# christopherkarani/Wax

Hardware: NVIDIA H100
Metric: queries/sec cosine top-10 @ 10Mx384 fp32 (higher is better)
Workload: dtype f32

## Files before the change

### wax_b200/csrc/waxvs_batch.cuh

```cuda
#pragma once
#include <cuda.h>
#include <cuda_bf16.h>

#include "waxvs_common.cuh"
#include "waxvs_scan.cuh"

namespace waxvs {

constexpr int kBatchM = 128;
constexpr int kBatchN = 128;
constexpr int kBatchKBlock = 32;
constexpr int kBatchKBlockBf16 = 64;
constexpr int kBatchRescore = 256;
constexpr int kBatchRescoreMax = 1024;
constexpr uint32_t kBatchABytes = kBatchM * 128u;
constexpr uint32_t kBatchBBytes = kBatchN * 128u;
constexpr uint32_t kBatchStageBytes = kBatchABytes + kBatchBBytes;
constexpr int kBatchStageSlots = 8;
constexpr uint32_t kBatchScoreStride = kBatchN + 8;
constexpr uint32_t kBatchScoreBytes = kBatchM * kBatchScoreStride * 4u;
constexpr int kBatchMaxStages = 6;
constexpr uint32_t kBatchSmemOptin = 227u * 1024u;
__host__ __device__ constexpr uint32_t batch_smem_bytes(int stages, int heap, uint32_t ares_kb = 0) {
    return ares_kb * kBatchABytes + stages * (ares_kb ? kBatchBBytes : kBatchStageBytes) + kBatchScoreBytes +
// ... 590 lines not shown
}

template <int METRIC>
__device__ __forceinline__ float exact_row_distance(const float *q, const float *v, uint32_t dims, float a2,
                                                    float sqrt_a2, int lane) {
    float a0 = 0.f, a1 = 0.f, a2_ = 0.f, a3 = 0.f, b0 = 0.f, b1 = 0.f, b2 = 0.f, b3 = 0.f;
    auto acc = [&](float qx, float vx, float &a, float &b) {
        if (METRIC == kL2) { const float dd = __fsub_rn(qx, vx); a = __fmaf_rn(dd, dd, a); }
        else { a = __fmaf_rn(qx, vx, a); if (METRIC == kCosine) b = __fmaf_rn(vx, vx, b); }
    };
    if ((dims % 4u) == 0u) {
        const float4 *v4 = reinterpret_cast<const float4 *>(v);
        const float4 *q4 = reinterpret_cast<const float4 *>(q);
        for (uint32_t c = lane; c < dims / 4u; c += 32u) {
            const float4 x = __ldg(v4 + c), y = __ldg(q4 + c);
            acc(y.x, x.x, a0, b0); acc(y.y, x.y, a1, b1); acc(y.z, x.z, a2_, b2); acc(y.w, x.w, a3, b3);
        }
    } else {
        for (uint32_t base = 4u * lane; base < dims; base += 128u) {
            acc(__ldg(q + base), __ldg(v + base), a0, b0);
            if (base + 1 < dims) acc(__ldg(q + base + 1), __ldg(v + base + 1), a1, b1);
            if (base + 2 < dims) acc(__ldg(q + base + 2), __ldg(v + base + 2), a2_, b2);
            if (base + 3 < dims) acc(__ldg(q + base + 3), __ldg(v + base + 3), a3, b3);
        }
    }
    const float s0 = warp_butterfly_sum(__fadd_rn(__fadd_rn(a0, a1), __fadd_rn(a2_, a3)));
    if (METRIC == kCosine) {
        const float s1 = warp_butterfly_sum(__fadd_rn(__fadd_rn(b0, b1), __fadd_rn(b2, b3)));
        return finish_cos(s0, a2, sqrt_a2, s1);
    }
    return METRIC == kDot ? finish_dot(s0) : finish_l2(s0);
}

template <int METRIC>
__device__ __forceinline__ void exact_row_distance_x4(const float *q, const float *const (&v)[4], uint32_t dims, float a2,
                                                      float sqrt_a2, int lane, float (&d)[4]) {
    if ((dims % 4u) != 0u) {
#pragma unroll
        for (int r = 0; r < 4; ++r) d[r] = exact_row_distance<METRIC>(q, v[r], dims, a2, sqrt_a2, lane);
        return;
    }
    float a[4][4], b[4][4];
#pragma unroll
    for (int r = 0; r < 4; ++r)
#pragma unroll
        for (int j = 0; j < 4; ++j) { a[r][j] = 0.f; b[r][j] = 0.f; }
    auto acc = [&](float qx, float vx, float &aa, float &bb) {
        if (METRIC == kL2) { const float dd = __fsub_rn(qx, vx); aa = __fmaf_rn(dd, dd, aa); }
        else { aa = __fmaf_rn(qx, vx, aa); if (METRIC == kCosine) bb = __fmaf_rn(vx, vx, bb); }
    };
    const float4 *q4 = reinterpret_cast<const float4 *>(q);
    for (uint32_t c = lane; c < dims / 4u; c += 32u) {
        float4 x[4];
#pragma unroll
        for (int r = 0; r < 4; ++r) x[r] = __ldg(reinterpret_cast<const float4 *>(v[r]) + c);
        const float4 y = __ldg(q4 + c);
#pragma unroll
        for (int r = 0; r < 4; ++r) {
            acc(y.x, x[r].x, a[r][0], b[r][0]); acc(y.y, x[r].y, a[r][1], b[r][1]);
            acc(y.z, x[r].z, a[r][2], b[r][2]); acc(y.w, x[r].w, a[r][3], b[r][3]);
        }
    }
#pragma unroll
    for (int r = 0; r < 4; ++r) {
        const float s0 = warp_butterfly_sum(__fadd_rn(__fadd_rn(a[r][0], a[r][1]), __fadd_rn(a[r][2], a[r][3])));
        if (METRIC == kCosine) {
            const float s1 = warp_butterfly_sum(__fadd_rn(__fadd_rn(b[r][0], b[r][1]), __fadd_rn(b[r][2], b[r][3])));
            d[r] = finish_cos(s0, a2, sqrt_a2, s1);
        } else {
            d[r] = METRIC == kDot ? finish_dot(s0) : finish_l2(s0);
        }
    }
}

__device__ __forceinline__ void block_bitonic_sort(uint64_t *sk, uint32_t pow2) {
    for (uint32_t size = 2; size <= pow2; size <<= 1) {
        for (uint32_t stride = size >> 1; stride > 0; stride >>= 1) {
            for (uint32_t i = threadIdx.x; i < pow2 / 2; i += blockDim.x) {
                const uint32_t lo = (i / stride) * (2 * stride) + (i % stride), hi = lo + stride;
                const bool asc = ((lo & size) == 0);
                const uint64_t a = sk[lo], b = sk[hi];
                if ((a > b) == asc) { sk[lo] = b; sk[hi] = a; }
            }
            __syncthreads();
        }
    }
}

template <int METRIC>
__global__ void __launch_bounds__(256) gather_score_kernel(const float *corpus, const float *queries, uint32_t dims,
                                                           const uint32_t *rows_all, const uint2 *span, uint32_t key_stride,
                                                           uint64_t *keys_all) {
    const int lane = threadIdx.x & 31;
// ... 105 lines not shown
                                         float eps_rel, bool excluded_any, uint32_t &ok, float &tau_star,
                                         float &tau_star16) {
    const float n = static_cast<float>(dims);
    const float delta = (n + 4.0f) * 0x1p-23f;
    const float one_m = __fsub_rd(1.0f, delta), one_p = __fadd_ru(1.0f, delta);
    const float qn = __fmul_ru(sqrt_a2, one_p);
    const float em = l2_nomination_bound(eps_rel, qn, max_norm, n);
    const float a_lo = __fsub_rd(__fmul_rd(a2, one_m), 1e-30f);
    float lhs = __fsub_rd(a_lo, __fmul_ru(2.0f, __fadd_ru(tau, em)));
    lhs = __fsub_rd(__fmul_rd(__fmul_rd(lhs, one_m), __fsub_rd(1.0f, 0x1p-20f)), 1e-30f);
    if (excluded_any && (!(lhs > dk) || !finite_f32(lhs) || !finite_f32(em) || !finite_f32(a2))) ok = 0;
    const float a_lo_f = __fsub_rd(__fdiv_rd(a2, one_p), 1e-30f);
    const float d_hi = __fadd_ru(__fdiv_ru(dk, one_m), 1e-30f);
    auto threshold = [&](float eps) {
        const float e = l2_nomination_bound(eps, qn, max_norm, n);
        const float t = __fsub_rd(__fmul_rd(0.5f, __fsub_rd(a_lo_f, d_hi)), e);
        return (finite_f32(t) && finite_f32(e) && finite_f32(a2)) ? t - fabsf(t) * 0x1p-20f - 1e-30f : -INFINITY;
    };
    tau_star = threshold(kTf32Eps);
    tau_star16 = threshold(kBf16Eps);
}

template <int METRIC>
__global__ void __launch_bounds__(512, 2) batch_finish_kernel(const FinishParams p) {
    extern __shared__ uint64_t fsm[];
    uint64_t *sk = fsm;
    uint64_t *ek = fsm + p.pow2_all;
    __shared__ float s_a2, s_sqrt_a2;
    __shared__ uint32_t s_valid, s_excl;
    const uint32_t q = blockIdx.x, g = q / kBatchM, t = q % kBatchM;
    const int warp = threadIdx.x >> 5, lane = threadIdx.x & 31;
    const float *qv = p.queries + static_cast<size_t>(q) * p.dims;

    if (threadIdx.x == 0) { s_valid = 0; s_excl = 0; }
    __syncthreads();
    const uint32_t total = p.slices * p.kprime;
    uint32_t cnt = 0;
    for (uint32_t i = threadIdx.x; i < p.pow2_all; i += blockDim.x) {
        uint64_t key = WAXVS_KEY_NONE;
        if (i < total) {
            const uint32_t s = i / p.kprime, e = i % p.kprime;
            key = p.heaps[(static_cast<size_t>(s * p.groups + g) * p.kprime + e) * kBatchM + t];
            if (key != WAXVS_KEY_NONE) {
                ++cnt;
                if (e == 0) atomicMax(&s_excl, orderable_u32(nominee_score(key)));
            }
        }
        sk[i] = key;
    }
    if (cnt) atomicAdd(&s_valid, cnt);
    if (warp == 0) {
        float s0 = 0.f, s1 = 0.f, s2 = 0.f, s3 = 0.f;
        for (uint32_t base = 4u * lane; base < p.dims; base += 128u) {
            const float x = __ldg(qv + base); s0 = __fmaf_rn(x, x, s0);
            if (base + 1 < p.dims) { const float y = __ldg(qv + base + 1); s1 = __fmaf_rn(y, y, s1); }
            if (base + 2 < p.dims) { const float z = __ldg(qv + base + 2); s2 = __fmaf_rn(z, z, s2); }
            if (base + 3 < p.dims) { const float w = __ldg(qv + base + 3); s3 = __fmaf_rn(w, w, s3); }
        }
        const float a2 = warp_butterfly_sum(__fadd_rn(__fadd_rn(s0, s1), __fadd_rn(s2, s3)));
        if (lane == 0) { s_a2 = a2; s_sqrt_a2 = __fsqrt_rn(a2); }
    }
    __syncthreads();
    block_bitonic_sort(sk, p.pow2_all);

    const uint32_t n_valid = s_valid;
    const uint32_t kpp = min(p.rescore, n_valid);
    float tau = s_excl ? from_orderable_u32(s_excl) : -INFINITY;
// ... 55 lines not shown
            ok = 0;
        }
        if (METRIC != kL2 && (!(s_a2 >= 0x1p-126f) || !finite_f32(s_a2))) {
            ok = 0;
            tau_star = tau_star16 = -INFINITY;
        }
        p.ok[q] = ok;
        if (p.tau_star) { p.tau_star[q] = tau_star; p.tau_star[p.tau_stride + q] = tau_star16; }
    }
    ScanParams sp{};
    sp.out = p.out + static_cast<size_t>(q) * p.k;
    sp.frame_ids = p.frame_ids; sp.id_base = p.id_base; sp.row_offset = p.row_offset;
    for (uint32_t i = threadIdx.x; i < p.k; i += blockDim.x)
        write_candidate(sp, static_cast<int>(i), i < p.rescore ? ek[i] : WAXVS_KEY_NONE);
}

struct RescoreParams {
    const float *corpus, *query;
    uint32_t dims, k, n_nominees;
    const uint64_t *nominees;
    uint32_t *aux;
    const uint32_t *max_norm_bits;
    float rho_max;
    uint64_t *block_keys;
    uint32_t *ticket;
    uint32_t *work_counter;
    wax_vs_candidate *out;
    uint32_t *ok;
    const uint64_t *frame_ids;
    uint64_t id_base, row_offset;
    uint32_t tail_smem_bytes;
};

template <int METRIC>
__global__ void __launch_bounds__(512, 1) shadow_rescore_kernel(const RescoreParams p) {
    static_assert(METRIC == kCosine || METRIC == kDot, "the shadow route covers cosine and dot");
    extern __shared__ __align__(16) unsigned char rsm[];
    __shared__ float s_a2, s_sqrt_a2;
    const int warp = threadIdx.x >> 5, lane = threadIdx.x & 31, warps = blockDim.x >> 5;
    const int k = static_cast<int>(p.k);
    if (warp == 0) {
        float s0 = 0.f, s1 = 0.f, s2 = 0.f, s3 = 0.f;
        for (uint32_t base = 4u * lane; base < p.dims; base += 128u) {
            const float4 x = __ldg(reinterpret_cast<const float4 *>(p.query + base));
            s0 = __fmaf_rn(x.x, x.x, s0); s1 = __fmaf_rn(x.y, x.y, s1);
            s2 = __fmaf_rn(x.z, x.z, s2); s3 = __fmaf_rn(x.w, x.w, s3);
        }
        const float a2 = warp_butterfly_sum(__fadd_rn(__fadd_rn(s0, s1), __fadd_rn(s2, s3)));
        if (lane == 0) { s_a2 = a2; s_sqrt_a2 = __fsqrt_rn(a2); }
    }
    __shared__ ScanParams sp;
    for (uint32_t i = threadIdx.x; i < sizeof(ScanParams) / 4u; i += blockDim.x) reinterpret_cast<uint32_t *>(&sp)[i] = 0u;
    __syncthreads();
    if (threadIdx.x == 0) {
        sp.k = p.k; sp.block_keys = p.block_keys; sp.ticket = p.ticket; sp.out = p.out;
        sp.frame_ids = p.frame_ids; sp.id_base = p.id_base; sp.row_offset = p.row_offset;
        sp.tail_smem_bytes = p.tail_smem_bytes; sp.work_counter = p.work_counter;
    }
    __syncthreads();

    WarpTopK<1> tk;
    tk.init();
    const uint32_t stride = gridDim.x * warps * 4u;
    for (uint32_t i0 = (blockIdx.x * warps + warp) * 4u; i0 < p.n_nominees; i0 += stride) {
        uint64_t nk[4];
        const float *vp[4];
        float d[4];
#pragma unroll
        for (uint32_t r = 0; r < 4; ++r) {
            nk[r] = i0 + r < p.n_nominees ? p.nominees[i0 + r] : WAXVS_KEY_NONE;
            vp[r] = p.corpus + static_cast<size_t>(nk[r] == WAXVS_KEY_NONE ? 0u : static_cast<uint32_t>(nk[r])) * p.dims;
        }
        exact_row_distance_x4<METRIC>(p.query, vp, p.dims, s_a2, s_sqrt_a2, lane, d);
#pragma unroll
        for (uint32_t r = 0; r < 4; ++r) {
            if (nk[r] == WAXVS_KEY_NONE || !finite_f32(d[r])) continue;
            const uint64_t x = make_key(d[r], static_cast<uint32_t>(nk[r]));
            if (x < tk.thresh) tk.insert(x, lane, k);
        }
    }

    if (!finish_topk_select<1>(sp, tk, rsm)) return;
    __syncthreads();
    if (threadIdx.x != 0) return;
    const wax_vs_candidate kth = p.out[p.k - 1];
    const uint32_t cut = p.aux[0];
    const bool excluded_any = cut != WAXVS_UKEY_NONE;
    const float tau = excluded_any ? -from_orderable_u32(cut) : -INFINITY;
    const float rho_q = __uint_as_float(p.aux[1]);
    uint32_t ok = 1;
    if (kth.valid) {
        const float dk = kth.distance, qn = s_sqrt_a2;
        const float m = METRIC == kCosine ? 1.0f : __uint_as_float(*p.max_norm_bits);
        const float scale = qn * m;
        const float sk_exact = METRIC == kCosine ? (1.0f - dk) * qn : 1.0f - dk;
        const float coding = qn * p.rho_max + rho_q * ((METRIC == kCosine ? 1.0001f : m) + p.rho_max);
        const float acc_slack = static_cast<float>(p.dims) * 0x1p-23f * scale;
        const float ulp_slack = 0x1p-21f * fmaxf(1.0f, fabsf(dk)) * (METRIC == kCosine ? qn : 1.0f);
        const float eps = coding * 1.01f + acc_slack + ulp_slack + 1e-30f;
        if (excluded_any && (!(sk_exact > tau + eps) || !finite_f32(eps))) ok = 0;
    } else if (excluded_any) {
        ok = 0;
    }
    if (!(s_a2 >= 0x1p-126f) || !finite_f32(s_a2)) ok = 0;
    *p.ok = ok;
    p.aux[0] = WAXVS_UKEY_NONE;
    p.aux[2] = cut;
}

template <int METRIC>
__global__ void __launch_bounds__(256) filter_rescore_kernel(const float *corpus, const float *queries, uint32_t dims,
                                                             const uint32_t *cand_count, const uint32_t *cand_rows,
// ... 71 lines not shown
```

### wax_b200/csrc/waxvs_common.cuh

```cuda
#pragma once
#include <cuda_runtime.h>
#include <stdint.h>

#define WAXVS_KEY_NONE 0xFFFFFFFFFFFFFFFFull
#define WAXVS_UKEY_NONE 0xFFFFFFFFu
#define WAXVS_FULL_MASK 0xFFFFFFFFu

namespace waxvs {

enum Metric : int { kCosine = 0, kDot = 1, kL2 = 2 };

__device__ __forceinline__ uint32_t orderable_u32(float f) {
    uint32_t u = __float_as_uint(f);
    return u ^ ((u & 0x80000000u) ? 0xFFFFFFFFu : 0x80000000u);
}
__device__ __forceinline__ float from_orderable_u32(uint32_t k) {
    uint32_t u = k ^ ((k & 0x80000000u) ? 0x80000000u : 0xFFFFFFFFu);
    return __uint_as_float(u);
}
__host__ __device__ __forceinline__ bool finite_f32(float f) {
#ifdef __CUDA_ARCH__
    return (__float_as_uint(f) & 0x7F800000u) != 0x7F800000u;
#else
    union { float f; uint32_t u; } x; x.f = f;
// ... 225 lines not shown
            "selp.u32 %0, 1, 0, p;\n\t}"
            : "=r"(done)
            : "r"(addr), "r"(parity)
            : "memory");
    } while (!done);
}
__device__ __forceinline__ void bulk_copy_g2s(void *smem_dst, const void *gmem_src, uint32_t bytes,
                                              uint64_t *bar) {
    asm volatile(
        "cp.async.bulk.shared::cluster.global.mbarrier::complete_tx::bytes [%0], [%1], %2, [%3];" ::"r"(
            smem_u32(smem_dst)),
        "l"(gmem_src), "r"(bytes), "r"(smem_u32(bar))
        : "memory");
}
__device__ __forceinline__ void bulk_copy_g2s_hint(void *smem_dst, const void *gmem_src, uint32_t bytes,
                                                   uint64_t *bar, uint64_t policy) {
    asm volatile(
        "cp.async.bulk.shared::cluster.global.mbarrier::complete_tx::bytes.L2::cache_hint [%0], [%1], %2, "
        "[%3], %4;" ::"r"(smem_u32(smem_dst)),
        "l"(gmem_src), "r"(bytes), "r"(smem_u32(bar)), "l"(policy)
        : "memory");
}
__device__ __forceinline__ uint64_t l2_policy_evict_first() {
    uint64_t pol;
    asm volatile("createpolicy.fractional.L2::evict_first.b64 %0, 1.0;" : "=l"(pol));
    return pol;
}
__device__ __forceinline__ uint64_t ld_cg_u64(const uint64_t *p) {
    uint64_t v;
    asm volatile("ld.global.cg.u64 %0, [%1];" : "=l"(v) : "l"(p) : "memory");
    return v;
}

}
```

### wax_b200/csrc/waxvs_engine.cu

```cuda
#include <cuda_runtime.h>

#include <algorithm>
#include <atomic>
#include <cstdarg>
#include <cstdio>
#include <cstring>
#include <limits>
#include <map>
#include <mutex>
#include <new>
#include <shared_mutex>
#include <string>
#include <unordered_map>
#include <chrono>
#include <random>
#include <thread>
#include <unistd.h>
#include <cmath>
#include <vector>

#include "../../include/wax_vs_cuda.h"
#include "waxvs_common.cuh"
#include "waxvs_scan.cuh"
#include "waxvs_select.cuh"
// ... 113 lines not shown
enum RouteForm : int { kRouteBf16, kRouteInt8, kRouteU4, kRouteForms };

struct Tuning {
    int variant = 0;
    int rows_per_step = 0;
    int stages = 0;
    int warps = 0;
    int grid = 0;
    int l2_hint = 0;
    int ldg_ctas_per_sm = 4;
    int chunk_steps = -1;
    int fused_k_max = 128;
    int batch_tensor = 1;
    int batch_min = 4;
    int time_overlap = 0;
    int batch_pair = 0;
    uint32_t tma_max_dims = 4096;
    int batch_large_k = 1;
    int batch_heap = 0;
    int batch_noinsert = 0;
    int batch_bf16 = 1;
    int batch_ares = 1;
    int batch_rescore = 0;
    int batch_retry = 1;
    int filter_bf16 = 1;
    int filter_cap = 8192;
    int inline_query = 1;
    int host_delivery = 1;
    int tail_select = 1;
    int shard_fused = 1;
    int batch_l2 = 0;
    int single_shadow = 0;
    uint64_t filter_bitset_bytes = 2ull << 30;
    int shadow_scan = 1;
    struct Route { uint64_t min_bytes; int rows_per_step = 0, warps = 0, stages = 0; };
    Route route[kRouteForms] = {
        {512ull << 20},
        {512ull << 20},
        {2048ull << 20},
    };
};

struct SearchCtx {
    cudaStream_t stream = nullptr;
    bool own_stream = false;
    DevBuf<float> d_queries;
    DevBuf<wax_vs_candidate> d_out;
    PinnedBuf<float> h_queries;
    PinnedBuf<wax_vs_candidate> h_out;
    DevBuf<uint64_t> d_block_keys;
    DevBuf<uint32_t> d_ticket;
    DevBuf<uint32_t> d_dist_keys;
    DevBuf<SelectState> d_select;
    DevBuf<uint64_t> d_sel_keys;
    cudaEvent_t ev0 = nullptr, ev1 = nullptr;
    DevBuf<uint64_t> d_heaps;
    DevBuf<uint32_t> d_ok;
    PinnedBuf<uint32_t> h_ok;
    DevBuf<uint32_t> d_tau;
    DevBuf<__nv_bfloat16> d_queries_bf16;
    DevBuf<float> d_retry_q;
    DevBuf<wax_vs_candidate> d_retry_out;
    DevBuf<uint32_t> d_retry_ok;
    DevBuf<float> d_tau_star;
    PinnedBuf<float> h_tau_star;
    DevBuf<float> d_filter_tau;
// ... 335 lines not shown
    } else if (C == 12) {
        R = e->tune.rows_per_step == 1 || e->tune.rows_per_step == 2 ? e->tune.rows_per_step : 2;
    } else if (C >= 6) {
        R = e->tune.rows_per_step == 2 || e->tune.rows_per_step == 4 ? e->tune.rows_per_step : 2;
    } else {
        R = e->tune.rows_per_step == 4 || e->tune.rows_per_step == 8 ? e->tune.rows_per_step : (C <= 2 ? 8 : 4);
        if (C == 1) warps_default = 16;
        else if (C == 2) warps_default = 12;
        else if (mode == 1 && static_cast<uint64_t>(e->n_rows) * d * 4 < (8ull << 30)) warps_default = 16;
    }
    const int stages = e->tune.stages > 0 ? e->tune.stages : 2;
    const size_t stage_bytes = static_cast<size_t>(R) * d * sizeof(float);
    const size_t query_bytes = C == 0 ? (static_cast<size_t>(d) * 4 + 512 + 32) : 0;
    auto smem_for = [&](int w) { return tma_ring_smem(w, stages, stage_bytes) + query_bytes; };
    int warps = std::max(1, std::min(16, e->tune.warps ? e->tune.warps : warps_default));
    if (!e->tune.warps) while (warps > 2 && smem_for(warps) > budget) --warps;
    if (smem_for(warps) > budget) return false;
    cfg->C = C; cfg->R = R; cfg->warps = warps; cfg->stages = stages; cfg->smem = smem_for(warps);
    return true;
}

template <typename K>
static cudaError_t grant_smem(wax_vs_engine *e, K kernel, size_t bytes) {
    static std::mutex mu;
    static std::map<std::pair<int, const void *>, int> granted;
    std::lock_guard<std::mutex> g(mu);
    int &have = granted[{e->device, reinterpret_cast<const void *>(kernel)}];
    if (have >= static_cast<int>(bytes)) return cudaSuccess;
    cudaError_t err = cudaFuncSetAttribute(kernel, cudaFuncAttributeMaxDynamicSharedMemorySize, static_cast<int>(bytes));
    if (err == cudaSuccess) have = static_cast<int>(bytes);
    return err;
}

template <int C, int R, int M, int E, bool EMIT, bool SHADOW = false, bool INT8 = false, bool U4 = false>
static cudaError_t launch_tma_inst(wax_vs_engine *e, const ScanParams &p, int grid, const TmaConfig &cfg, cudaStream_t s) {
    cudaError_t err = grant_smem(e, scan_tma_kernel<C, R, M, E, EMIT, SHADOW, INT8, U4>, cfg.smem);
    if (err != cudaSuccess) return err;
    scan_tma_kernel<C, R, M, E, EMIT, SHADOW, INT8, U4><<<grid, cfg.warps * 32, cfg.smem, s>>>(p);
    return cudaGetLastError();
}
template <int C, int R>
static cudaError_t launch_tma_cr(wax_vs_engine *e, const ScanParams &p, int grid, const TmaConfig &cfg, int metric, int mode,
                                 cudaStream_t s) {
    switch (metric * 3 + mode) {
        case 0: return launch_tma_inst<C, R, kCosine, 1, false>(e, p, grid, cfg, s);
        case 1: return launch_tma_inst<C, R, kCosine, 4, false>(e, p, grid, cfg, s);
        case 2: return launch_tma_inst<C, R, kCosine, 1, true>(e, p, grid, cfg, s);
        case 3: return launch_tma_inst<C, R, kDot, 1, false>(e, p, grid, cfg, s);
        case 4: return launch_tma_inst<C, R, kDot, 4, false>(e, p, grid, cfg, s);
        case 5: return launch_tma_inst<C, R, kDot, 1, true>(e, p, grid, cfg, s);
        case 6: return launch_tma_inst<C, R, kL2, 1, false>(e, p, grid, cfg, s);
        case 7: return launch_tma_inst<C, R, kL2, 4, false>(e, p, grid, cfg, s);
        default: return launch_tma_inst<C, R, kL2, 1, true>(e, p, grid, cfg, s);
    }
}
static cudaError_t launch_tma(wax_vs_engine *e, const ScanParams &p, int grid, const TmaConfig &cfg, int metric, int mode,
                              cudaStream_t s) {
#define WAXVS_CASE(Cv, Rv) if (cfg.C == Cv && cfg.R == Rv) return launch_tma_cr<Cv, Rv>(e, p, grid, cfg, metric, mode, s)
    WAXVS_CASE(1, 4); WAXVS_CASE(1, 8); WAXVS_CASE(2, 4); WAXVS_CASE(2, 8);
    WAXVS_CASE(3, 4); WAXVS_CASE(3, 8); WAXVS_CASE(4, 4); WAXVS_CASE(4, 8);
    WAXVS_CASE(6, 2); WAXVS_CASE(6, 4); WAXVS_CASE(8, 2); WAXVS_CASE(8, 4);
    WAXVS_CASE(12, 1); WAXVS_CASE(12, 2);
    WAXVS_CASE(0, 1); WAXVS_CASE(0, 2); WAXVS_CASE(0, 4); WAXVS_CASE(0, 8);
#undef WAXVS_CASE
    return cudaErrorInvalidValue;
}
template <RouteForm F, int C, int R>
static cudaError_t launch_route_cr(wax_vs_engine *e, const ScanParams &p, int grid, const TmaConfig &cfg, int metric,
                                   cudaStream_t s) {
    if constexpr (F == kRouteU4) {
        return launch_tma_inst<C, R, kDot, 4, false, true, false, true>(e, p, grid, cfg, s);
    } else {
        return metric == kCosine ? launch_tma_inst<C, R, kCosine, 4, false, true, F == kRouteInt8>(e, p, grid, cfg, s)
                                 : launch_tma_inst<C, R, kDot, 4, false, true, F == kRouteInt8>(e, p, grid, cfg, s);
    }
}
#define WAXVS_CASE(Cv, Rv) \
    if (cfg.C == Cv && cfg.R == Rv) return p ? launch_route_cr<F, Cv, Rv>(e, *p, grid, cfg, metric, s) : cudaSuccess
static cudaError_t launch_shadow_scan(wax_vs_engine *e, const ScanParams *p, int grid, const TmaConfig &cfg, int metric,
                                      cudaStream_t s) {
    constexpr RouteForm F = kRouteBf16;
    WAXVS_CASE(1, 8); WAXVS_CASE(1, 16); WAXVS_CASE(2, 8); WAXVS_CASE(2, 16);
    WAXVS_CASE(3, 4); WAXVS_CASE(3, 8); WAXVS_CASE(3, 16); WAXVS_CASE(4, 4); WAXVS_CASE(4, 8);
    WAXVS_CASE(6, 2); WAXVS_CASE(6, 4); WAXVS_CASE(8, 2); WAXVS_CASE(8, 4); WAXVS_CASE(12, 2); WAXVS_CASE(12, 4);
    return cudaErrorInvalidValue;
}
static cudaError_t launch_int8_scan(wax_vs_engine *e, const ScanParams *p, int grid, const TmaConfig &cfg, int metric,
                                   cudaStream_t s) {
    constexpr RouteForm F = kRouteInt8;
    WAXVS_CASE(1, 8); WAXVS_CASE(1, 16); WAXVS_CASE(2, 8); WAXVS_CASE(2, 16);
    WAXVS_CASE(3, 4); WAXVS_CASE(3, 8); WAXVS_CASE(3, 16); WAXVS_CASE(4, 4); WAXVS_CASE(4, 8);
// ... 143 lines not shown

static bool batch_bf16_wanted(const wax_vs_engine *e);
static int32_t ensure_shadow(wax_vs_engine *e, cudaStream_t stream);
static int32_t ensure_coded_shadow(wax_vs_engine *e, RouteForm f, cudaStream_t stream, bool keep_coarse);
static int32_t ensure_route_shadow(wax_vs_engine *e, RouteForm f, cudaStream_t stream, bool keep_coarse = false) {
    return f == kRouteBf16 ? ensure_shadow(e, stream) : ensure_coded_shadow(e, f, stream, keep_coarse);
}

constexpr uint32_t kShadowNominees = 128;
constexpr uint32_t kShadowRescore = 256;
constexpr uint32_t kShadowSkipQueries = 16;
static bool shadow_route_applies(const wax_vs_engine *e) {
    return e->tune.shadow_scan && (e->similarity == WAX_VS_COSINE || e->similarity == WAX_VS_DOT) && !e->debug_trace &&
           e->tune.batch_bf16 != 0 && e->dims % kBatchKBlockBf16 == 0 &&
           e->n_rows * e->dims * sizeof(float) >= e->tune.route[kRouteBf16].min_bytes;
}
static int32_t select_route_form(wax_vs_engine *e, cudaStream_t stream, bool demoted, bool *use, RouteForm *form,
                                 TmaConfig *cfg) {
    *use = false;
    for (const RouteForm f : {kRouteU4, kRouteInt8, kRouteBf16}) {
        if ((f == kRouteU4 && demoted) || e->n_rows * e->dims * sizeof(float) < e->tune.route[f].min_bytes ||
            !pick_route_config(e, f, cfg))
            continue;
        if (const int32_t rc = ensure_route_shadow(e, f, stream)) return rc;
        if (e->shadows[f].valid && e->shadows[f].eps_rel <= kRouteSpec[f].max_eps_rel) {
            *use = true;
            *form = f;
            return WAX_VS_OK;
        }
    }
    return WAX_VS_OK;
}

static int32_t enqueue_shadow_nominations(wax_vs_engine *e, SearchCtx *c, const ScanParams &p, const TmaConfig &cfg,
                                          cudaStream_t stream, uint64_t *launches, uint32_t *shape, RouteForm f) {
    const RouteFormSpec &fs = kRouteSpec[f];
    const wax_vs_engine::Shadow &sh = e->shadows[f];
    int32_t rc;
    if (fs.grid_rescore && !c->d_u4_aux) {
        if ((rc = c->d_u4_aux.ensure(3, "4-bit route state"))) return rc;
        CUDA_TRY(cudaMemsetAsync(c->d_u4_aux, 0xFF, 3 * sizeof(uint32_t), stream));
    }
    const size_t cta_keys = static_cast<size_t>(std::max(e->tune.grid, e->sm_count)) * kU4CtaNominees;
    if ((rc = c->d_heaps.ensure(std::max(static_cast<size_t>(kShadowNominees) * kNomineeStride, fs.grid_rescore ? cta_keys : 0), "nominee keys")) ||
        (rc = c->d_ok.ensure(1, "proof flags")) || (!p.query && (rc = c->d_queries.ensure(e->dims, "query buffer"))))
        return rc;

    ScanParams sp = p;
    sp.corpus = reinterpret_cast<const float *>(sh.codes.p);
    sp.row_scale = fs.scaled ? sh.scale.p : nullptr;
    sp.u4_aux = fs.grid_rescore ? c->d_u4_aux.p : nullptr;
    sp.k = kShadowNominees;
    sp.out = nullptr; sp.host_out = nullptr; sp.host_flag = nullptr;
    sp.nominees = c->d_heaps;
    sp.query_store = p.query ? nullptr : c->d_queries.p;
    sp.tail_select = e->tune.tail_select ? 1u : 0u;
    sp.tail_smem_bytes = static_cast<uint32_t>(static_cast<size_t>(cfg.warps) * cfg.stages * cfg.R * e->dims * fs.tail_bytes);
    const int grid = tma_grid(e, c, cfg, sp);
    CUDA_TRY(fs.launch(e, &sp, grid, cfg, e->similarity, stream));

    if (fs.grid_rescore) {
        RescoreParams rp{};
        rp.corpus = e->d_corpus; rp.query = p.query ? p.query : c->d_queries.p;
        rp.dims = e->dims; rp.k = p.k; rp.n_nominees = static_cast<uint32_t>(grid) * kU4CtaNominees;
        rp.nominees = c->d_heaps; rp.aux = c->d_u4_aux; rp.max_norm_bits = e->d_max_norm; rp.rho_max = sh.rho_max;
        rp.block_keys = c->d_block_keys; rp.ticket = c->d_ticket; rp.work_counter = sp.work_counter; rp.out = p.out; rp.ok = c->d_ok;
        rp.frame_ids = p.frame_ids; rp.id_base = p.id_base; rp.row_offset = p.row_offset;
        rp.tail_smem_bytes = static_cast<uint32_t>(grid) * p.k * sizeof(uint64_t);
        if (rp.tail_smem_bytes > 48u * 1024u) rp.tail_smem_bytes = 0;
        const auto kernel = e->similarity == WAX_VS_COSINE ? shadow_rescore_kernel<kCosine> : shadow_rescore_kernel<kDot>;
        kernel<<<grid, 512, rp.tail_smem_bytes, stream>>>(rp);
        CUDA_TRY(cudaGetLastError());
    } else {
        FinishParams fp{};
        fp.corpus = e->d_corpus; fp.queries = p.query ? p.query : c->d_queries.p;
        fp.n_rows = p.n_rows; fp.dims = e->dims; fp.n_queries = 1; fp.groups = 1; fp.slices = 1;
        fp.kprime = kShadowNominees; fp.k = p.k; fp.metric = e->similarity;
        fp.heaps = c->d_heaps; fp.max_norm_bits = e->d_max_norm;
        fp.out = p.out; fp.ok = c->d_ok;
        fp.frame_ids = p.frame_ids; fp.id_base = p.id_base; fp.row_offset = p.row_offset;
        fp.pow2_all = 512; fp.rescore = kShadowRescore; fp.eps_rel = sh.eps_rel;
        const size_t fsmem = static_cast<size_t>(fp.pow2_all + fp.rescore) * sizeof(uint64_t);
        const auto kernel = e->similarity == WAX_VS_COSINE ? batch_finish_kernel<kCosine> : batch_finish_kernel<kDot>;
        CUDA_TRY(grant_smem(e, kernel, fsmem));
        kernel<<<1, 512, fsmem, stream>>>(fp);
        CUDA_TRY(cudaGetLastError());
    }
    *launches += 2;
    if (shape) {
        const uint32_t s[7] = {static_cast<uint32_t>(cfg.C), static_cast<uint32_t>(cfg.R), static_cast<uint32_t>(cfg.warps),
                               static_cast<uint32_t>(cfg.stages), static_cast<uint32_t>(grid), sp.chunk_steps, sp.tail_select};
        std::copy(s, s + 7, shape);
    }
    return WAX_VS_OK;
}

static int32_t enqueue_shadow_route(wax_vs_engine *e, SearchCtx *c, ScanParams &p, cudaStream_t stream, uint64_t *launches) {
    if (!shadow_route_applies(e)) return WAX_VS_OK;
    int32_t rc;
    if (!c->h_proof_count) {
        if ((rc = c->d_proof_count.ensure(2, "proof counts")) || (rc = c->h_proof_count.ensure(2, "proof count mirror"))) return rc;
        CUDA_TRY(cudaMemsetAsync(c->d_proof_count, 0, 2 * sizeof(uint32_t), stream));
        c->h_proof_count[0] = c->h_proof_count[1] = 0;
        c->seen_failed = 0;
    }
    bool demoted;
    {
        std::lock_guard<std::mutex> pg(e->pool_mu);
        const uint32_t failed = *static_cast<volatile uint32_t *>(c->h_proof_count + 1);
        if (failed != c->seen_failed) {
            c->seen_failed = failed;
            if (c->last_u4) {
                if (e->u4_probing) e->u4_demote_window = std::min(e->u4_demote_window * 2, 1u << 20);
                e->u4_demoted = e->u4_demote_window;
            } else {
                e->shadow_scan_skip = kShadowSkipQueries;
            }
        } else if (c->last_u4 && e->u4_probing) {
            e->u4_demote_window = 16;
// ... 89 lines not shown
    }

    TmaConfig cfg{};
    bool use_tma = (e->tune.variant != 2) && pick_tma_config(e, &cfg, mode);
    if (e->tune.variant == 1 && !use_tma)
        return fail(WAX_VS_ERR_UNSUPPORTED, "TMA-staged kernel does not support dims=%u", e->dims);
    if (host && host->h_query) {
        int32_t rc = place_host_query(e, c, p, host->h_query, use_tma && !emit, stream);
        if (rc) return rc;
    }
    if (host && host->host_out && !emit && !shard) {
        p.host_out = host->host_out; p.host_flag = host->host_flag; p.host_seq = host->seq;
        const_cast<HostDelivery *>(host)->delivered = true;
    }
    if (use_tma && !emit && e->tune.tail_select) {
        p.tail_select = 1u;
        p.tail_smem_bytes = static_cast<uint32_t>(static_cast<size_t>(cfg.warps) * cfg.stages * cfg.R * e->dims * sizeof(float));
    }
    bool fused_exchange = false;
    if (shard && !emit) {
        const size_t list_bytes = p.tail_select ? p.tail_smem_bytes
                                                : static_cast<size_t>(use_tma ? cfg.warps : 8) * 32 * (mode == 0 ? 1 : 4) * sizeof(uint64_t);
        fused_exchange = e->tune.shard_fused != 0 && static_cast<size_t>(shard->world) * k_eff * sizeof(uint32_t) <= list_bytes;
        if (fused_exchange) { p.shard = *shard; p.shard.final_out = d_merged; }
    }
    if (shadow_route && !shard && mode == 0 && use_tma && cfg.C > 0) {
        int32_t rc = enqueue_shadow_route(e, c, p, stream, launches);
        if (rc) return rc;
    }
    int grid;
    const int grid_cap = static_cast<int>(c->d_block_keys.cap / 128);
    if (use_tma) {
        grid = tma_grid(e, c, cfg, p);
        CUDA_TRY(launch_tma(e, p, grid, cfg, e->similarity, mode, stream));
    } else {
        const int max_grid = e->tune.grid > 0 ? e->tune.grid : e->sm_count * e->tune.ldg_ctas_per_sm;
        grid = static_cast<int>(std::min<uint64_t>(max_grid, (e->n_rows + 7) / 8));
        grid = std::max(std::min(grid, grid_cap), 1);
        CUDA_TRY(launch_ldg(p, grid, e->similarity, mode, stream));
    }
    ++*launches;

    if (emit && !keys_only) {
        int32_t rc = enqueue_select(e, c, c->d_dist_keys, static_cast<uint32_t>(e->n_rows), k_eff, p, stream, launches);
        if (rc) return rc;
    }
    if (shard && !fused_exchange) return exchange_standalone();
    return WAX_VS_OK;
}

static PFN_cuTensorMapEncodeTiled_v12000 tensor_map_encoder() {
    static PFN_cuTensorMapEncodeTiled_v12000 fn = nullptr;
    static std::once_flag once;
    std::call_once(once, [] {
        void *ptr = nullptr;
        cudaDriverEntryPointQueryResult q;
        if (cudaGetDriverEntryPoint("cuTensorMapEncodeTiled", &ptr, cudaEnableDefault, &q) == cudaSuccess &&
            q == cudaDriverEntryPointSuccess)
            fn = reinterpret_cast<PFN_cuTensorMapEncodeTiled_v12000>(ptr);
    });
    return fn;
}

static int32_t make_tensor_map(CUtensorMap *map, const void *base, uint64_t rows, uint32_t dims, uint32_t box_rows,
                               bool bf16 = false) {
    auto enc = tensor_map_encoder();
    if (!enc) return fail(WAX_VS_ERR_CUDA, "cuTensorMapEncodeTiled is not available from this driver");
// ... 4037 lines not shown
    else if (!strcmp(key, "filter_bitset_bytes")) e->tune.filter_bitset_bytes = static_cast<uint64_t>(std::max<int64_t>(value, 0));
    else if (!strcmp(key, "single_shadow")) e->tune.single_shadow = v;
    else if (!strcmp(key, "shadow_scan")) {
        std::lock_guard<std::mutex> pg(e->pool_mu);
        e->tune.shadow_scan = v;
        e->shadow_scan_skip = 0;
        auto seen = [](SearchCtx *c) { if (c->h_proof_count) c->seen_failed = *static_cast<volatile uint32_t *>(c->h_proof_count + 1); };
        for (SearchCtx *c : e->pool) seen(c);
        for (auto &kv : e->stream_ctx) seen(kv.second);
    }
    else if (!strcmp(key, "shadow_rows_per_step")) e->tune.route[kRouteBf16].rows_per_step = v;
    else if (!strcmp(key, "shadow_warps")) e->tune.route[kRouteBf16].warps = v;
    else if (!strcmp(key, "shadow_stages")) e->tune.route[kRouteBf16].stages = v;
    else if (!strcmp(key, "shadow_scan_min_bytes")) e->tune.route[kRouteBf16].min_bytes = static_cast<uint64_t>(std::max<int64_t>(value, 0));
    else if (!strcmp(key, "int8_scan_min_bytes")) {
        e->tune.route[kRouteInt8].min_bytes = static_cast<uint64_t>(std::max<int64_t>(value, 0));
        e->shadows[kRouteInt8].unavailable = false;
        e->shadows[kRouteInt8].coarse = false;
    }
    else if (!strcmp(key, "u4_scan_min_bytes")) {
        e->tune.route[kRouteU4].min_bytes = static_cast<uint64_t>(std::max<int64_t>(value, 0));
        e->shadows[kRouteU4].unavailable = false;
        e->shadows[kRouteU4].coarse = false;
        e->u4_demoted = 0; e->u4_demote_window = 16; e->u4_probing = false;
    }
    else if (!strcmp(key, "u4_rows_per_step")) e->tune.route[kRouteU4].rows_per_step = v;
    else if (!strcmp(key, "u4_warps")) e->tune.route[kRouteU4].warps = v;
    else if (!strcmp(key, "u4_stages")) e->tune.route[kRouteU4].stages = v;
    else if (!strcmp(key, "int8_rows_per_step")) e->tune.route[kRouteInt8].rows_per_step = v;
    else if (!strcmp(key, "int8_warps")) e->tune.route[kRouteInt8].warps = v;
    else if (!strcmp(key, "int8_stages")) e->tune.route[kRouteInt8].stages = v;
    else if (!strcmp(key, "shard_fused")) e->tune.shard_fused = v;
    else if (!strcmp(key, "tail_select")) e->tune.tail_select = v;
    else if (!strcmp(key, "inline_query")) e->tune.inline_query = v;
    else if (!strcmp(key, "host_delivery")) e->tune.host_delivery = v;
    else if (!strcmp(key, "shard_timeout_ms")) e->shard.timeout_ns = static_cast<unsigned long long>(std::max<int64_t>(value, 1)) * 1000000ull;
    else if (!strcmp(key, "time_overlap")) e->tune.time_overlap = v;
    else if (!strcmp(key, "ldg_ctas_per_sm")) e->tune.ldg_ctas_per_sm = std::max(1, v);
    else return fail(WAX_VS_ERR_ARGUMENT, "unknown option '%s'", key);
    return WAX_VS_OK;
}

}
```

### wax_b200/csrc/waxvs_scan.cuh

```cuda
#pragma once
#include "waxvs_common.cuh"
#include "waxvs_shard.cuh"
#include "../../include/wax_vs_cuda.h"

namespace waxvs {

constexpr int kInlineQueryFloats = 512;

struct ScanParams {
    const float *corpus;
    const float *query;
    uint32_t n_rows;
    uint32_t dims;
    uint32_t k;
    uint32_t stages;
    uint64_t *block_keys;
    uint32_t *ticket;
    wax_vs_candidate *out;
    uint32_t *dist_keys;
    const uint64_t *frame_ids;
    uint64_t id_base;
    uint64_t row_offset;
    uint32_t use_l2_hint;
    uint32_t chunk_steps;
// ... 271 lines not shown
    __shared__ SelectScratch ss;
    __shared__ uint32_t s_cut;
    const uint32_t tid = threadIdx.x, nthr = blockDim.x;
    if (tid == 0) s_cut = WAXVS_UKEY_NONE;
    auto own_keys = [&](auto f) {
#pragma unroll
        for (int j = 0; j < E; ++j) f(tk.key[j]);
    };
    const uint64_t xa = nthr * E >= kU4CtaNominees ? block_select_kth(own_keys, kU4CtaNominees, &ss) : WAXVS_KEY_NONE;
    if (tid == 0) ss.n_sel = 0;
    __syncthreads();
    uint64_t *mine = p.nominees + static_cast<size_t>(blockIdx.x) * kU4CtaNominees;
#pragma unroll
    for (int j = 0; j < E; ++j)
        if (tk.key[j] != WAXVS_KEY_NONE && tk.key[j] <= xa) mine[atomicAdd(&ss.n_sel, 1u)] = tk.key[j];
    if ((tid & 31u) == 0 && tk.thresh != WAXVS_KEY_NONE) atomicMin(&s_cut, static_cast<uint32_t>(tk.thresh >> 32));
    __syncthreads();
    for (uint32_t i = ss.n_sel + tid; i < kU4CtaNominees; i += nthr) mine[i] = WAXVS_KEY_NONE;
    if (tid == 0) {
        uint32_t cut = s_cut;
        if (xa != WAXVS_KEY_NONE) cut = min(cut, static_cast<uint32_t>(xa >> 32));
        if (cut != WAXVS_UKEY_NONE) atomicMin(p.u4_aux, cut);
    }
}

template <int C, int R, int METRIC, int E, bool EMIT, bool SHADOW = false, bool INT8 = false, bool U4 = false>
__global__ void __launch_bounds__(512, 1) scan_tma_kernel(const __grid_constant__ ScanParams p) {
    static_assert(!SHADOW || (C > 0 && METRIC != kL2 && !EMIT), "the shadow form covers the unrolled cosine / dot shapes");
    static_assert(!INT8 || (SHADOW && R >= 4), "the int8 form is a shadow form with 16-byte scale copies");
    static_assert(!U4 || (SHADOW && !INT8 && R >= 4 && E == 4), "the 4-bit form is a shadow form with 16-byte scale copies");
    constexpr bool SCALED = INT8 || U4;
    if constexpr (!SHADOW && !EMIT && E == 1 && METRIC != kL2) {
        if (p.proof_ok) {
            const bool proven = *p.proof_ok != 0u;
            if (blockIdx.x == 0) {
                if (threadIdx.x == 0) {
                    const uint32_t n = ++p.proof_count[proven ? 0 : 1];
                    *static_cast<volatile uint32_t *>(p.proof_count_host + (proven ? 0 : 1)) = n;
                }
                if (proven && p.host_flag) {
                    for (uint32_t i = threadIdx.x; i < p.k; i += blockDim.x) p.host_out[i] = p.out[i];
                    __threadfence_system();
                    __syncthreads();
                    if (threadIdx.x == 0) st_release_sys_u64(p.host_flag, p.host_seq);
                }
            }
            if (proven) return;
        }
    }
    const int D4 = C > 0 ? 32 * C : static_cast<int>(p.dims / 4u);
    const int CN = C > 0 ? C : (D4 + 31) / 32;
    const uint32_t ROW_BYTES = C > 0 ? (U4 ? 64u : INT8 ? 128u : SHADOW ? 256u : 512u) * C : p.dims * 4u;
    const uint32_t STAGE_BYTES = ROW_BYTES * R + (SCALED ? R * 4u : 0u);
    constexpr int LANES_PER_ROW = 32 / R;

    extern __shared__ __align__(128) unsigned char smem[];
    const int warp = threadIdx.x >> 5, lane = threadIdx.x & 31, warps = blockDim.x >> 5;
    const uint32_t stages = p.stages;
    unsigned char *ring = smem + static_cast<size_t>(warp) * stages * STAGE_BYTES;
    uint64_t *bars = reinterpret_cast<uint64_t *>(smem + static_cast<size_t>(warps) * stages * STAGE_BYTES) +
                     warp * stages;
    uint64_t *lists = reinterpret_cast<uint64_t *>(smem + static_cast<size_t>(warps) * stages * STAGE_BYTES) +
                      warps * stages;
    uint32_t *stage_step = reinterpret_cast<uint32_t *>(lists + warps * 32 * E) + warp * stages;
    float4 *qs = reinterpret_cast<float4 *>(reinterpret_cast<uint32_t *>(lists + warps * 32 * E) + warps * stages + 4);

// ... 244 lines not shown
        else if (METRIC == kCosine) d = finish_cos(sum0[0], a2, sqrt_a2, sum1[0]);
        else if (METRIC == kDot) d = finish_dot(sum0[0]);
        else d = finish_l2(sum0[0]);
        if (SHADOW && !finite_f32(d)) d = -INFINITY;
        const bool leader = U4 ? (hl % (16 / H)) == 0 : (lane % LANES_PER_ROW) == 0;
        const bool ok = (my_row < p.n_rows) && (SHADOW || finite_f32(d));

        if (EMIT) {
            if (leader && my_row < p.n_rows)
                p.dist_keys[my_row] = (ok && row_allowed(p, my_row)) ? orderable_u32(d) : WAXVS_UKEY_NONE;
        } else {
            const uint64_t key = ok ? make_key(d, my_row) : WAXVS_KEY_NONE;
            const bool cand = leader && key < tk.thresh && row_allowed(p, my_row);
            uint32_t m = __ballot_sync(WAXVS_FULL_MASK, cand);
            if (E == 1) {
                while (m) {
                    const int src = __ffs(m) - 1;
                    m &= m - 1;
                    const uint64_t x = shfl_u64(key, src);
                    if (x < tk.thresh) tk.insert(x, lane, k);
                }
            } else if (m) {
                if (tk.npend + __popc(m) > 32) tk.flush(lane, k);
                while (m) {
                    const int src = __ffs(m) - 1;
                    m &= m - 1;
                    tk.park(shfl_u64(key, src), lane);
                }
            }
        }
    }

    if (p.trace && lane == 0) atomicMax(p.trace + 1, global_timer_ns());
    if (!EMIT) {
        if (E > 1) tk.flush(lane, k);
        if constexpr (U4) finish_u4_nominees<E>(p, tk);
        else if (p.tail_select) finish_topk_select<E, SHADOW>(p, tk, smem);
        else finish_topk<E, SHADOW>(p, tk, lists, warp, lane, warps);
    }
}

template <int METRIC, int E, bool EMIT>
__global__ void __launch_bounds__(256, 4) scan_ldg_kernel(const __grid_constant__ ScanParams p) {
    __shared__ uint64_t lists[8 * 32 * E];
    const int warp = threadIdx.x >> 5, lane = threadIdx.x & 31, warps = blockDim.x >> 5;
    const uint32_t dims = p.dims;
    const bool vec4 = (dims % 4u) == 0u;
    const uint32_t d4 = dims / 4u;

    float a2 = 0.0f, sqrt_a2 = 0.0f;
    if (METRIC == kCosine) {
        float s0 = 0.f, s1 = 0.f, s2 = 0.f, s3 = 0.f;
        for (uint32_t base = 4u * lane; base < dims; base += 128u) {
            const float x = __ldg(p.query + base);
            const float y = (base + 1 < dims) ? __ldg(p.query + base + 1) : 0.0f;
            const float z = (base + 2 < dims) ? __ldg(p.query + base + 2) : 0.0f;
            const float w = (base + 3 < dims) ? __ldg(p.query + base + 3) : 0.0f;
            s0 = __fmaf_rn(x, x, s0);
            if (base + 1 < dims) s1 = __fmaf_rn(y, y, s1);
            if (base + 2 < dims) s2 = __fmaf_rn(z, z, s2);
            if (base + 3 < dims) s3 = __fmaf_rn(w, w, s3);
        }
        a2 = warp_butterfly_sum(__fadd_rn(__fadd_rn(s0, s1), __fadd_rn(s2, s3)));
        sqrt_a2 = __fsqrt_rn(a2);
    }

// ... 61 lines not shown
```

Measured before the change: 1498.

## Chain shadow route kernels with programmatic dependent launch and specialise rescore by dims

Launches the rescore/finish kernels and the proof-gated fallback scan with programmatic stream serialization, so each kernel's prologue can overlap the tail of the previous one. Kernels call griddepcontrol.wait before reading upstream results. The shadow rescore kernel is also templated on a compile-time chunk count for common dims, which fully unrolls the loads. Every warp now computes the query norm itself instead of waiting on warp 0, and the next nominee keys are prefetched one iteration ahead. The change adds a launch-path dependency on PDL support, and correctness depends on every wait being placed before the first read of upstream data.

```diff
diff --git a/wax_b200/csrc/waxvs_batch.cuh b/wax_b200/csrc/waxvs_batch.cuh
--- a/wax_b200/csrc/waxvs_batch.cuh
+++ b/wax_b200/csrc/waxvs_batch.cuh
@@ -646,7 +646,7 @@
     return METRIC == kDot ? finish_dot(s0) : finish_l2(s0);
 }
 
-template <int METRIC>
+template <int METRIC, int CC = 0>
 __device__ __forceinline__ void exact_row_distance_x4(const float *q, const float *const (&v)[4], uint32_t dims, float a2,
                                                       float sqrt_a2, int lane, float (&d)[4]) {
     if ((dims % 4u) != 0u) {
@@ -664,15 +664,32 @@
         else { aa = __fmaf_rn(qx, vx, aa); if (METRIC == kCosine) bb = __fmaf_rn(vx, vx, bb); }
     };
     const float4 *q4 = reinterpret_cast<const float4 *>(q);
-    for (uint32_t c = lane; c < dims / 4u; c += 32u) {
-        float4 x[4];
-#pragma unroll
-        for (int r = 0; r < 4; ++r) x[r] = __ldg(reinterpret_cast<const float4 *>(v[r]) + c);
-        const float4 y = __ldg(q4 + c);
-#pragma unroll
-        for (int r = 0; r < 4; ++r) {
-            acc(y.x, x[r].x, a[r][0], b[r][0]); acc(y.y, x[r].y, a[r][1], b[r][1]);
-            acc(y.z, x[r].z, a[r][2], b[r][2]); acc(y.w, x[r].w, a[r][3], b[r][3]);
+    if constexpr (CC > 0) {
+        float4 x[CC][4];
+#pragma unroll
+        for (int c = 0; c < CC; ++c)
+#pragma unroll
+            for (int r = 0; r < 4; ++r) x[c][r] = __ldg(reinterpret_cast<const float4 *>(v[r]) + lane + 32 * c);
+#pragma unroll
+        for (int c = 0; c < CC; ++c) {
+            const float4 y = __ldg(q4 + lane + 32 * c);
+#pragma unroll
+            for (int r = 0; r < 4; ++r) {
+                acc(y.x, x[c][r].x, a[r][0], b[r][0]); acc(y.y, x[c][r].y, a[r][1], b[r][1]);
+                acc(y.z, x[c][r].z, a[r][2], b[r][2]); acc(y.w, x[c][r].w, a[r][3], b[r][3]);
+            }
+        }
+    } else {
+        for (uint32_t c = lane; c < dims / 4u; c += 32u) {
+            float4 x[4];
+#pragma unroll
+            for (int r = 0; r < 4; ++r) x[r] = __ldg(reinterpret_cast<const float4 *>(v[r]) + c);
+            const float4 y = __ldg(q4 + c);
+#pragma unroll
+            for (int r = 0; r < 4; ++r) {
+                acc(y.x, x[r].x, a[r][0], b[r][0]); acc(y.y, x[r].y, a[r][1], b[r][1]);
+                acc(y.z, x[r].z, a[r][2], b[r][2]); acc(y.w, x[r].w, a[r][3], b[r][3]);
+            }
         }
     }
 #pragma unroll
@@ -844,7 +861,9 @@
     const int warp = threadIdx.x >> 5, lane = threadIdx.x & 31;
     const float *qv = p.queries + static_cast<size_t>(q) * p.dims;
 
+    pdl_launch_dependents();
     if (threadIdx.x == 0) { s_valid = 0; s_excl = 0; }
+    pdl_wait();
     __syncthreads();
     const uint32_t total = p.slices * p.kprime;
     uint32_t cnt = 0;
@@ -966,23 +985,14 @@
     uint32_t tail_smem_bytes;
 };
 
-template <int METRIC>
+template <int METRIC, int CC>
 __global__ void __launch_bounds__(512, 1) shadow_rescore_kernel(const RescoreParams p) {
     static_assert(METRIC == kCosine || METRIC == kDot, "the shadow route covers cosine and dot");
     extern __shared__ __align__(16) unsigned char rsm[];
     __shared__ float s_a2, s_sqrt_a2;
     const int warp = threadIdx.x >> 5, lane = threadIdx.x & 31, warps = blockDim.x >> 5;
     const int k = static_cast<int>(p.k);
-    if (warp == 0) {
-        float s0 = 0.f, s1 = 0.f, s2 = 0.f, s3 = 0.f;
-        for (uint32_t base = 4u * lane; base < p.dims; base += 128u) {
-            const float4 x = __ldg(reinterpret_cast<const float4 *>(p.query + base));
-            s0 = __fmaf_rn(x.x, x.x, s0); s1 = __fmaf_rn(x.y, x.y, s1);
-            s2 = __fmaf_rn(x.z, x.z, s2); s3 = __fmaf_rn(x.w, x.w, s3);
-        }
-        const float a2 = warp_butterfly_sum(__fadd_rn(__fadd_rn(s0, s1), __fadd_rn(s2, s3)));
-        if (lane == 0) { s_a2 = a2; s_sqrt_a2 = __fsqrt_rn(a2); }
-    }
+    pdl_launch_dependents();
     __shared__ ScanParams sp;
     for (uint32_t i = threadIdx.x; i < sizeof(ScanParams) / 4u; i += blockDim.x) reinterpret_cast<uint32_t *>(&sp)[i] = 0u;
     __syncthreads();
@@ -992,26 +1002,53 @@
         sp.tail_smem_bytes = p.tail_smem_bytes; sp.work_counter = p.work_counter;
     }
     __syncthreads();
+    pdl_wait();
+    float a2, sqrt_a2;
+    {
+        float s0 = 0.f, s1 = 0.f, s2 = 0.f, s3 = 0.f;
+        auto sq = [&](float4 x) {
+            s0 = __fmaf_rn(x.x, x.x, s0); s1 = __fmaf_rn(x.y, x.y, s1);
+            s2 = __fmaf_rn(x.z, x.z, s2); s3 = __fmaf_rn(x.w, x.w, s3);
+        };
+        if constexpr (CC > 0) {
+            float4 x[CC];
+#pragma unroll
+            for (int c = 0; c < CC; ++c) x[c] = __ldg(reinterpret_cast<const float4 *>(p.query) + lane + 32 * c);
+#pragma unroll
+            for (int c = 0; c < CC; ++c) sq(x[c]);
+        } else {
+            for (uint32_t base = 4u * lane; base < p.dims; base += 128u) sq(__ldg(reinterpret_cast<const float4 *>(p.query + base)));
+        }
+        a2 = warp_butterfly_sum(__fadd_rn(__fadd_rn(s0, s1), __fadd_rn(s2, s3)));
+        sqrt_a2 = __fsqrt_rn(a2);
+        if (warp == 0 && lane == 0) { s_a2 = a2; s_sqrt_a2 = sqrt_a2; }
+    }
 
     WarpTopK<1> tk;
     tk.init();
     const uint32_t stride = gridDim.x * warps * 4u;
+    auto nominee = [&](uint32_t i) { return i < p.n_nominees ? p.nominees[i] : WAXVS_KEY_NONE; };
+    uint64_t nk[4];
+#pragma unroll
+    for (uint32_t r = 0; r < 4; ++r) nk[r] = nominee((blockIdx.x * warps + warp) * 4u + r);
     for (uint32_t i0 = (blockIdx.x * warps + warp) * 4u; i0 < p.n_nominees; i0 += stride) {
-        uint64_t nk[4];
         const float *vp[4];
         float d[4];
+        uint64_t next[4];
 #pragma unroll
         for (uint32_t r = 0; r < 4; ++r) {
-            nk[r] = i0 + r < p.n_nominees ? p.nominees[i0 + r] : WAXVS_KEY_NONE;
             vp[r] = p.corpus + static_cast<size_t>(nk[r] == WAXVS_KEY_NONE ? 0u : static_cast<uint32_t>(nk[r])) * p.dims;
-        }
-        exact_row_distance_x4<METRIC>(p.query, vp, p.dims, s_a2, s_sqrt_a2, lane, d);
+            next[r] = nominee(i0 + stride + r);
+        }
+        exact_row_distance_x4<METRIC, CC>(p.query, vp, p.dims, a2, sqrt_a2, lane, d);
 #pragma unroll
         for (uint32_t r = 0; r < 4; ++r) {
             if (nk[r] == WAXVS_KEY_NONE || !finite_f32(d[r])) continue;
             const uint64_t x = make_key(d[r], static_cast<uint32_t>(nk[r]));
             if (x < tk.thresh) tk.insert(x, lane, k);
         }
+#pragma unroll
+        for (uint32_t r = 0; r < 4; ++r) nk[r] = next[r];
     }
 
     if (!finish_topk_select<1>(sp, tk, rsm)) return;
diff --git a/wax_b200/csrc/waxvs_common.cuh b/wax_b200/csrc/waxvs_common.cuh
--- a/wax_b200/csrc/waxvs_common.cuh
+++ b/wax_b200/csrc/waxvs_common.cuh
@@ -281,4 +281,7 @@
     return v;
 }
 
-}
+__device__ __forceinline__ void pdl_wait() { asm volatile("griddepcontrol.wait;" ::: "memory"); }
+__device__ __forceinline__ void pdl_launch_dependents() { asm volatile("griddepcontrol.launch_dependents;" ::: "memory"); }
+
+}
diff --git a/wax_b200/csrc/waxvs_engine.cu b/wax_b200/csrc/waxvs_engine.cu
--- a/wax_b200/csrc/waxvs_engine.cu
+++ b/wax_b200/csrc/waxvs_engine.cu
@@ -169,6 +169,7 @@
     int batch_l2 = 0;
     int single_shadow = 0;
     uint64_t filter_bitset_bytes = 2ull << 30;
+    int route_pdl = 1;
     int shadow_scan = 1;
     struct Route { uint64_t min_bytes; int rows_per_step = 0, warps = 0, stages = 0; };
     Route route[kRouteForms] = {
@@ -570,21 +571,34 @@
     return err;
 }
 
+template <typename... Args>
+static cudaError_t launch_maybe_chained(bool chain, void (*kernel)(Args...), int grid, int threads, size_t smem,
+                                        cudaStream_t s, const Args &...args) {
+    cudaLaunchAttribute attr{};
+    attr.id = cudaLaunchAttributeProgrammaticStreamSerialization;
+    attr.val.programmaticStreamSerializationAllowed = 1;
+    cudaLaunchConfig_t lc{};
+    lc.gridDim = dim3(grid); lc.blockDim = dim3(threads); lc.dynamicSmemBytes = smem; lc.stream = s;
+    lc.attrs = chain ? &attr : nullptr;
+    lc.numAttrs = chain ? 1 : 0;
+    return cudaLaunchKernelEx(&lc, kernel, args...);
+}
+
 template <int C, int R, int M, int E, bool EMIT, bool SHADOW = false, bool INT8 = false, bool U4 = false>
-static cudaError_t launch_tma_inst(wax_vs_engine *e, const ScanParams &p, int grid, const TmaConfig &cfg, cudaStream_t s) {
+static cudaError_t launch_tma_inst(wax_vs_engine *e, const ScanParams &p, int grid, const TmaConfig &cfg, cudaStream_t s,
+                                   bool chain = false) {
     cudaError_t err = grant_smem(e, scan_tma_kernel<C, R, M, E, EMIT, SHADOW, INT8, U4>, cfg.smem);
     if (err != cudaSuccess) return err;
-    scan_tma_kernel<C, R, M, E, EMIT, SHADOW, INT8, U4><<<grid, cfg.warps * 32, cfg.smem, s>>>(p);
-    return cudaGetLastError();
+    return launch_maybe_chained(chain, scan_tma_kernel<C, R, M, E, EMIT, SHADOW, INT8, U4>, grid, cfg.warps * 32, cfg.smem, s, p);
 }
 template <int C, int R>
 static cudaError_t launch_tma_cr(wax_vs_engine *e, const ScanParams &p, int grid, const TmaConfig &cfg, int metric, int mode,
-                                 cudaStream_t s) {
+                                 cudaStream_t s, bool chain) {
     switch (metric * 3 + mode) {
-        case 0: return launch_tma_inst<C, R, kCosine, 1, false>(e, p, grid, cfg, s);
+        case 0: return launch_tma_inst<C, R, kCosine, 1, false>(e, p, grid, cfg, s, chain);
         case 1: return launch_tma_inst<C, R, kCosine, 4, false>(e, p, grid, cfg, s);
         case 2: return launch_tma_inst<C, R, kCosine, 1, true>(e, p, grid, cfg, s);
-        case 3: return launch_tma_inst<C, R, kDot, 1, false>(e, p, grid, cfg, s);
+        case 3: return launch_tma_inst<C, R, kDot, 1, false>(e, p, grid, cfg, s, chain);
         case 4: return launch_tma_inst<C, R, kDot, 4, false>(e, p, grid, cfg, s);
         case 5: return launch_tma_inst<C, R, kDot, 1, true>(e, p, grid, cfg, s);
         case 6: return launch_tma_inst<C, R, kL2, 1, false>(e, p, grid, cfg, s);
@@ -593,8 +607,8 @@
     }
 }
 static cudaError_t launch_tma(wax_vs_engine *e, const ScanParams &p, int grid, const TmaConfig &cfg, int metric, int mode,
-                              cudaStream_t s) {
-#define WAXVS_CASE(Cv, Rv) if (cfg.C == Cv && cfg.R == Rv) return launch_tma_cr<Cv, Rv>(e, p, grid, cfg, metric, mode, s)
+                              cudaStream_t s, bool chain = false) {
+#define WAXVS_CASE(Cv, Rv) if (cfg.C == Cv && cfg.R == Rv) return launch_tma_cr<Cv, Rv>(e, p, grid, cfg, metric, mode, s, chain)
     WAXVS_CASE(1, 4); WAXVS_CASE(1, 8); WAXVS_CASE(2, 4); WAXVS_CASE(2, 8);
     WAXVS_CASE(3, 4); WAXVS_CASE(3, 8); WAXVS_CASE(4, 4); WAXVS_CASE(4, 8);
     WAXVS_CASE(6, 2); WAXVS_CASE(6, 4); WAXVS_CASE(8, 2); WAXVS_CASE(8, 4);
@@ -804,6 +818,16 @@
     return WAX_VS_OK;
 }
 
+static void (*rescore_kernel(bool cosine, uint32_t dims))(RescoreParams) {
+    switch (dims) {
+        case 128: return cosine ? shadow_rescore_kernel<kCosine, 1> : shadow_rescore_kernel<kDot, 1>;
+        case 256: return cosine ? shadow_rescore_kernel<kCosine, 2> : shadow_rescore_kernel<kDot, 2>;
+        case 384: return cosine ? shadow_rescore_kernel<kCosine, 3> : shadow_rescore_kernel<kDot, 3>;
+        case 512: return cosine ? shadow_rescore_kernel<kCosine, 4> : shadow_rescore_kernel<kDot, 4>;
+        default: return cosine ? shadow_rescore_kernel<kCosine, 0> : shadow_rescore_kernel<kDot, 0>;
+    }
+}
+
 static int32_t enqueue_shadow_nominations(wax_vs_engine *e, SearchCtx *c, const ScanParams &p, const TmaConfig &cfg,
                                           cudaStream_t stream, uint64_t *launches, uint32_t *shape, RouteForm f) {
     const RouteFormSpec &fs = kRouteSpec[f];
@@ -840,9 +864,8 @@
         rp.frame_ids = p.frame_ids; rp.id_base = p.id_base; rp.row_offset = p.row_offset;
         rp.tail_smem_bytes = static_cast<uint32_t>(grid) * p.k * sizeof(uint64_t);
         if (rp.tail_smem_bytes > 48u * 1024u) rp.tail_smem_bytes = 0;
-        const auto kernel = e->similarity == WAX_VS_COSINE ? shadow_rescore_kernel<kCosine> : shadow_rescore_kernel<kDot>;
-        kernel<<<grid, 512, rp.tail_smem_bytes, stream>>>(rp);
-        CUDA_TRY(cudaGetLastError());
+        CUDA_TRY(launch_maybe_chained(e->tune.route_pdl != 0, rescore_kernel(e->similarity == WAX_VS_COSINE, e->dims), grid,
+                                      512, rp.tail_smem_bytes, stream, rp));
     } else {
         FinishParams fp{};
         fp.corpus = e->d_corpus; fp.queries = p.query ? p.query : c->d_queries.p;
@@ -855,8 +878,7 @@
         const size_t fsmem = static_cast<size_t>(fp.pow2_all + fp.rescore) * sizeof(uint64_t);
         const auto kernel = e->similarity == WAX_VS_COSINE ? batch_finish_kernel<kCosine> : batch_finish_kernel<kDot>;
         CUDA_TRY(grant_smem(e, kernel, fsmem));
-        kernel<<<1, 512, fsmem, stream>>>(fp);
-        CUDA_TRY(cudaGetLastError());
+        CUDA_TRY(launch_maybe_chained(e->tune.route_pdl != 0, kernel, 1, 512, fsmem, stream, fp));
     }
     *launches += 2;
     if (shape) {
@@ -1012,7 +1034,7 @@
     const int grid_cap = static_cast<int>(c->d_block_keys.cap / 128);
     if (use_tma) {
         grid = tma_grid(e, c, cfg, p);
-        CUDA_TRY(launch_tma(e, p, grid, cfg, e->similarity, mode, stream));
+        CUDA_TRY(launch_tma(e, p, grid, cfg, e->similarity, mode, stream, p.proof_ok != nullptr && e->tune.route_pdl != 0));
     } else {
         const int max_grid = e->tune.grid > 0 ? e->tune.grid : e->sm_count * e->tune.ldg_ctas_per_sm;
         grid = static_cast<int>(std::min<uint64_t>(max_grid, (e->n_rows + 7) / 8));
@@ -5116,6 +5138,7 @@
     else if (!strcmp(key, "int8_stages")) e->tune.route[kRouteInt8].stages = v;
     else if (!strcmp(key, "shard_fused")) e->tune.shard_fused = v;
     else if (!strcmp(key, "tail_select")) e->tune.tail_select = v;
+    else if (!strcmp(key, "route_pdl")) e->tune.route_pdl = v;
     else if (!strcmp(key, "inline_query")) e->tune.inline_query = v;
     else if (!strcmp(key, "host_delivery")) e->tune.host_delivery = v;
     else if (!strcmp(key, "shard_timeout_ms")) e->shard.timeout_ns = static_cast<unsigned long long>(std::max<int64_t>(value, 1)) * 1000000ull;
diff --git a/wax_b200/csrc/waxvs_scan.cuh b/wax_b200/csrc/waxvs_scan.cuh
--- a/wax_b200/csrc/waxvs_scan.cuh
+++ b/wax_b200/csrc/waxvs_scan.cuh
@@ -327,6 +327,7 @@
     constexpr bool SCALED = INT8 || U4;
     if constexpr (!SHADOW && !EMIT && E == 1 && METRIC != kL2) {
         if (p.proof_ok) {
+            pdl_wait();
             const bool proven = *p.proof_ok != 0u;
             if (blockIdx.x == 0) {
                 if (threadIdx.x == 0) {
@@ -637,6 +638,7 @@
     }
 
     if (p.trace && lane == 0) atomicMax(p.trace + 1, global_timer_ns());
+    if constexpr (SHADOW) pdl_launch_dependents();
     if (!EMIT) {
         if (E > 1) tk.flush(lane, k);
         if constexpr (U4) finish_u4_nominees<E>(p, tk);
```

Result: no change. 1510, median of 6 (+0.8%).
